# Aditya-Somasi/Vision-Inspection-System

Hardware: AMD Instinct MI355X
Metric: inspected images/sec (1024x1024, Qwen2-VL-7B) (higher is better)
Workload: dtype bf16; 1 GPU; configs[1]: Qwen2-VL-7B Inspector bf16, single 1024x1024 image per step per GPU, greedy decode 128 tok; batch=1, image_px=1024, weights=seeded random bf16 at exact 7B shapes, parallelism=dp1 (whole images)

## Files before the change

### vision-inspection-system_amd/csrc/decode.hip

```cpp
#include "decode_common.hip.h"
#include <stdlib.h>

template <int NB, bool AMAX, bool MASK>
__device__ __forceinline__ void gemv_bf16_body(GemvArgs p, const unsigned long long* __restrict__ allow) {
  extern __shared__ __attribute__((aligned(16))) char smem[];
  bf16_t* xs = (bf16_t*)smem;
  const int tid = threadIdx.x, lane = tid & 63, wave = tid >> 6;
  const int nch = p.K >> 3;

  const bool swiglu = (p.act == GV_ACT_SWIGLU);
  const int n_pairs = swiglu ? (p.N >> 1) : ((p.N + 1) >> 1);
  const int n_waves = gridDim.x * 4;
  const int wid = blockIdx.x * 4 + wave;
  const int p_begin = (int)((long long)n_pairs * wid / n_waves);
  const int p_end = (int)((long long)n_pairs * (wid + 1) / n_waves);
  const int nseg = ((nch + 63) / 64 + GV_SEG - 1) / GV_SEG;
  const int n_tasks = (p_end - p_begin) * nseg;

  GvBuf A, B;
  if (n_tasks > 0) gv_load(A, p, swiglu, p_begin, 0, lane, nch);

#pragma unroll
  for (int r = 0; r < NB; ++r) {
    if (r > 0) __syncthreads();
    gv_stage_row(p.x + (size_t)min(r, p.nb - 1) * p.ldx, p.norm_w, xs + (size_t)r * p.K, nch, p.K, p.eps, tid, lane, wave);
  }
  __syncthreads();

  float a0[NB], a1[NB];
#pragma unroll
  for (int r = 0; r < NB; ++r) { a0[r] = 0.f; a1[r] = 0.f; }
  float best = -INFINITY;
  int bi = 0x7fffffff;
  const unsigned am_step = AMAX ? (unsigned)*p.am_step : 0u;
  auto amax_rows = [&](int pr) {
    if (lane != 0) return;
    const int o = 2 * pr;
    float v0 = a0[0], v1 = a1[0];
    if (p.am_inv_temp > 0.f) {
      v0 = v0 * p.am_inv_temp + gumbel_noise(p.am_seed, am_step, (unsigned)o);
      v1 = v1 * p.am_inv_temp + gumbel_noise(p.am_seed, am_step, (unsigned)(o + 1));
    }
    bool ok0 = true, ok1 = true;
    if constexpr (MASK) {
      const unsigned long long m = allow[o >> 6];
      ok0 = (m >> (o & 63)) & 1ull;
      ok1 = (m >> ((o + 1) & 63)) & 1ull;
    }
    if (ok0 && (v0 > best || (v0 == best && o < bi))) { best = v0; bi = o; }
    if (ok1 && o + 1 < p.N && (v1 > best || (v1 == best && o + 1 < bi))) { best = v1; bi = o + 1; }
  };
  int pair = p_begin, seg = 0;
  for (int t = 0; t < n_tasks; t += 2) {
    int pair1 = pair, seg1 = seg + 1;
    if (seg1 == nseg) { seg1 = 0; ++pair1; }
    if (t + 1 < n_tasks) gv_load(B, p, swiglu, pair1, seg1, lane, nch);
    gv_consume<NB>(A, xs, p.K, seg, lane, nch, a0, a1);
    if (seg == nseg - 1) {
      gv_finish<NB>(p, swiglu, pair, lane, a0, a1);
      if constexpr (AMAX) amax_rows(pair);
#pragma unroll
      for (int r = 0; r < NB; ++r) { a0[r] = 0.f; a1[r] = 0.f; }
    }
    if (t + 1 >= n_tasks) break;
    int pair2 = pair1, seg2 = seg1 + 1;
    if (seg2 == nseg) { seg2 = 0; ++pair2; }
    if (t + 2 < n_tasks) gv_load(A, p, swiglu, pair2, seg2, lane, nch);
    gv_consume<NB>(B, xs, p.K, seg1, lane, nch, a0, a1);
    if (seg1 == nseg - 1) {
      gv_finish<NB>(p, swiglu, pair1, lane, a0, a1);
      if constexpr (AMAX) amax_rows(pair1);
#pragma unroll
      for (int r = 0; r < NB; ++r) { a0[r] = 0.f; a1[r] = 0.f; }
    }
    pair = pair2;
    seg = seg2;
  }
  if constexpr (AMAX) {
    __shared__ float am_v[4];
    __shared__ int am_i[4];
    if (lane == 0) { am_v[wave] = best; am_i[wave] = bi; }
    __syncthreads();
    if (tid == 0) {
      for (int w = 1; w < 4; ++w)
        if (am_v[w] > best || (am_v[w] == best && am_i[w] < bi)) { best = am_v[w]; bi = am_i[w]; }
      p.am_val[blockIdx.x] = best;
      p.am_idx[blockIdx.x] = bi;
    }
  }
}

template <int NB, bool AMAX = false>
__global__ __launch_bounds__(256) void gemv_bf16_kernel(GemvArgs p) { gemv_bf16_body<NB, AMAX, false>(p, nullptr); }

__global__ __launch_bounds__(256) void gemv_bf16_argmax_masked_kernel(GemvArgs p, const unsigned long long* allow) {
  gemv_bf16_body<1, true, true>(p, allow);
}

static int gemv_bf16_launch(GemvArgs p, hipStream_t stream) {
  const int n_pairs = (p.act == GV_ACT_SWIGLU) ? p.N / 2 : (p.N + 1) / 2;
  int blocks = (n_pairs + 3) / 4;
  if (blocks > 1024) blocks = 1024 + (blocks - 1024) / 8;
  if (blocks > 2048) blocks = 2048;
  vis_clear_error();
  if (p.nb == 1) {
    hipLaunchKernelGGL(gemv_bf16_kernel<1>, dim3(blocks), dim3(256), (size_t)p.K * 2, stream, p);
  } else {
    static const bool attr_ok = [] {
      return hipFuncSetAttribute((const void*)gemv_bf16_kernel<2>, hipFuncAttributeMaxDynamicSharedMemorySize, GV_ROWS_LDS_MAX) == hipSuccess &&
             hipFuncSetAttribute((const void*)gemv_bf16_kernel<4>, hipFuncAttributeMaxDynamicSharedMemorySize, GV_ROWS_LDS_MAX) == hipSuccess;
    }();
    if (!attr_ok) return VIS_ERR_LAUNCH;
    if (p.nb == 2) hipLaunchKernelGGL(gemv_bf16_kernel<2>, dim3(blocks), dim3(256), (size_t)p.K * 4, stream, p);
    else hipLaunchKernelGGL(gemv_bf16_kernel<4>, dim3(blocks), dim3(256), (size_t)p.K * 8, stream, p);
  }
  return vis_check_launch();
}

extern "C" int vis_gemv_bf16(const void* x, const void* W, const void* bias, const void* R, const void* norm_w,
                             void* y, int N, int K, int ldw, int act, int out_f32, float eps,
                             hipStream_t stream) {
  if (!x || !W || !y || N <= 0 || K <= 0) return VIS_ERR_ARG;
  if (K % 8 != 0 || ldw % 8 != 0 || K * 2 > 60 * 1024) return VIS_ERR_ARG;
  if (act != GV_ACT_NONE && act != GV_ACT_SWIGLU) return VIS_ERR_ARG;
  if (act == GV_ACT_SWIGLU && (N % 32 != 0 || bias || R || out_f32)) return VIS_ERR_ARG;
  if (((uintptr_t)x | (uintptr_t)W | (uintptr_t)norm_w) & 15) return VIS_ERR_ARG;
  GemvArgs p;
  p.x = (const bf16_t*)x; p.W = (const bf16_t*)W; p.bias = (const bf16_t*)bias; p.R = (const bf16_t*)R;
  p.norm_w = (const bf16_t*)norm_w; p.y = y;
  p.N = N; p.K = K; p.ldw = ldw; p.act = act; p.out_f32 = out_f32; p.eps = eps;
  p.outs_per_block = 0;
  p.nb = 1; p.ldx = 0; p.ldy = 0; p.ldr = 0;
  return gemv_bf16_launch(p, stream);
}

extern "C" int vis_gemv_bf16_rows(const void* x, const void* W, const void* bias, const void* R, const void* norm_w,
                                  void* y, int B, int N, int K, int ldw, int ldx, int ldy, int ldr, int act, int out_f32,
                                  float eps, hipStream_t stream) {
  if (!x || !W || !y || N <= 0 || K <= 0 || B < 1 || B > 4) return VIS_ERR_ARG;
  if (K % 8 != 0 || ldw % 8 != 0 || ldx % 8 != 0 || ldx < K) return VIS_ERR_ARG;
  const int nbk = (B == 1) ? 1 : (B == 2 ? 2 : 4);
  if ((size_t)K * 2 * nbk > (size_t)(nbk == 1 ? 60 * 1024 : GV_ROWS_LDS_MAX)) return VIS_ERR_ARG;
  if (act != GV_ACT_NONE && act != GV_ACT_SWIGLU) return VIS_ERR_ARG;
  if (act == GV_ACT_SWIGLU && (N % 32 != 0 || bias || R || out_f32)) return VIS_ERR_ARG;
  if (ldy < ((act == GV_ACT_SWIGLU) ? N / 2 : N) || (R && ldr < N)) return VIS_ERR_ARG;
  if (((uintptr_t)x | (uintptr_t)W | (uintptr_t)norm_w) & 15) return VIS_ERR_ARG;
  GemvArgs p;
  p.x = (const bf16_t*)x; p.W = (const bf16_t*)W; p.bias = (const bf16_t*)bias; p.R = (const bf16_t*)R;
  p.norm_w = (const bf16_t*)norm_w; p.y = y;
  p.N = N; p.K = K; p.ldw = ldw; p.act = act; p.out_f32 = out_f32; p.eps = eps;
  p.outs_per_block = 0;
  p.nb = B; p.ldx = ldx; p.ldy = ldy; p.ldr = ldr;
  return gemv_bf16_launch(p, stream);
}


struct GemvF8Args {
  const bf16_t* x;
  const uint8_t* W;
  const float* scale;
  const bf16_t* bias;
  const bf16_t* R;
  const bf16_t* norm_w;
  void* y;
  int N, K, ldw;
  int act, out_f32;
  float eps;
  int nb, ldx, ldy, ldr;
};

template <int ROWS, int SEG>
struct GfBuf {
  u32x4 w[ROWS][SEG];
};

template <int ROWS>
__device__ __forceinline__ void gf_rows(const GemvF8Args& p, bool swiglu, int quad, int* r) {
  if (swiglu) {
    const int o = (ROWS / 2) * quad;
    const int g0 = ((o >> 4) << 5) + (o & 15);
#pragma unroll
    for (int i = 0; i < ROWS / 2; ++i) { r[2 * i] = g0 + i; r[2 * i + 1] = g0 + 16 + i; }
  } else {
#pragma unroll
    for (int i = 0; i < ROWS; ++i) r[i] = min(ROWS * quad + i, p.N - 1);
  }
}

template <int ROWS, int SEG>
__device__ __forceinline__ void gf_load(GfBuf<ROWS, SEG>& b, const GemvF8Args& p, bool swiglu, int quad, int seg,
                                        int lane, int nch) {
  int r[ROWS];
  gf_rows<ROWS>(p, swiglu, quad, r);
#pragma unroll
  for (int i = 0; i < ROWS; ++i) {
    const uint8_t* w = p.W + (size_t)r[i] * p.ldw;
#pragma unroll
    for (int u = 0; u < SEG; ++u) {
      const int c = min(lane + 64 * (seg * SEG + u), nch - 1);
      b.w[i][u] = __builtin_nontemporal_load((const u32x4*)(w + c * 16));
    }
  }
}

struct Gf16 {
  bf16x2 v[8];
};
__device__ __forceinline__ Gf16 cvt16_f8(const u32x4& w) {
  Gf16 r;
#pragma unroll
  for (int i = 0; i < 4; ++i) {
    r.v[2 * i] = __builtin_amdgcn_cvt_scalef32_pk_bf16_fp8(w[i], 1.0f, false);
    r.v[2 * i + 1] = __builtin_amdgcn_cvt_scalef32_pk_bf16_fp8(w[i], 1.0f, true);
  }
  return r;
}
__device__ __forceinline__ float dot16_f8(const Gf16& w, const u32x4& xlo, const u32x4& xhi, float acc) {
  const bf16x8 xa = __builtin_bit_cast(bf16x8, xlo), xb = __builtin_bit_cast(bf16x8, xhi);
  acc = __builtin_amdgcn_fdot2_f32_bf16(w.v[0], __builtin_shufflevector(xa, xa, 0, 1), acc, false);
  acc = __builtin_amdgcn_fdot2_f32_bf16(w.v[1], __builtin_shufflevector(xa, xa, 2, 3), acc, false);
  acc = __builtin_amdgcn_fdot2_f32_bf16(w.v[2], __builtin_shufflevector(xa, xa, 4, 5), acc, false);
  acc = __builtin_amdgcn_fdot2_f32_bf16(w.v[3], __builtin_shufflevector(xa, xa, 6, 7), acc, false);
  acc = __builtin_amdgcn_fdot2_f32_bf16(w.v[4], __builtin_shufflevector(xb, xb, 0, 1), acc, false);
  acc = __builtin_amdgcn_fdot2_f32_bf16(w.v[5], __builtin_shufflevector(xb, xb, 2, 3), acc, false);
  acc = __builtin_amdgcn_fdot2_f32_bf16(w.v[6], __builtin_shufflevector(xb, xb, 4, 5), acc, false);
  acc = __builtin_amdgcn_fdot2_f32_bf16(w.v[7], __builtin_shufflevector(xb, xb, 6, 7), acc, false);
  return acc;
}

template <int ROWS, int SEG, int NB>
__device__ __forceinline__ void gf_consume(const GfBuf<ROWS, SEG>& b, const bf16_t* xs, int K, int seg, int lane, int nch,
                                           float (&a)[NB][ROWS]) {
#pragma unroll
  for (int u = 0; u < SEG; ++u) {
    const int c = lane + 64 * (seg * SEG + u);
    const int cc = min(c, nch - 1);
    u32x4 xlo[NB], xhi[NB];
#pragma unroll
    for (int r = 0; r < NB; ++r) {
      xlo[r] = *(const u32x4*)(xs + (size_t)r * K + cc * 16);
      xhi[r] = *(const u32x4*)(xs + (size_t)r * K + cc * 16 + 8);
      if (c >= nch) { xlo[r] = (u32x4){0u, 0u, 0u, 0u}; xhi[r] = xlo[r]; }
    }
#pragma unroll
    for (int i = 0; i < ROWS; ++i) {
      const Gf16 wv = cvt16_f8(b.w[i][u]);
#pragma unroll
      for (int r = 0; r < NB; ++r) a[r][i] = dot16_f8(wv, xlo[r], xhi[r], a[r][i]);
    }
  }
}

template <int ROWS, int NB>
__device__ __forceinline__ void gf_finish(const GemvF8Args& p, bool swiglu, int quad, int lane, float (&a)[NB][ROWS]) {
#pragma unroll
  for (int r = 0; r < NB; ++r)
#pragma unroll
    for (int i = 0; i < ROWS; ++i) a[r][i] = wave_sum(a[r][i]);
  if (lane != 0) return;
  int rw[ROWS];
  gf_rows<ROWS>(p, swiglu, quad, rw);
#pragma unroll
  for (int r = 0; r < NB; ++r) {
    if (r >= p.nb) break;
    if (swiglu) {
#pragma unroll
      for (int i = 0; i < ROWS / 2; ++i) {
        const float g = a[r][2 * i] * p.scale[rw[2 * i]], u = a[r][2 * i + 1] * p.scale[rw[2 * i + 1]];
        ((bf16_t*)p.y)[(size_t)r * p.ldy + (ROWS / 2) * quad + i] = f2bf(silu_fast(g) * u);
      }
      continue;
    }
#pragma unroll
    for (int i = 0; i < ROWS; ++i) {
      const int o = ROWS * quad + i;
      if (o >= p.N) break;
      float v = a[r][i] * p.scale[o];
      if (p.bias) v += bf2f(p.bias[o]);
      if (p.R) v += bf2f(p.R[(size_t)r * p.ldr + o]);
      if (p.out_f32) ((float*)p.y)[(size_t)r * p.ldy + o] = v;
      else ((bf16_t*)p.y)[(size_t)r * p.ldy + o] = f2bf(v);
    }
  }
}

template <int ROWS, int SEG, int NB>
__global__ __launch_bounds__(256) void gemv_fp8w_kernel(GemvF8Args p) {
  extern __shared__ __attribute__((aligned(16))) char smem[];
  bf16_t* xs = (bf16_t*)smem;
  const int tid = threadIdx.x, lane = tid & 63, wave = tid >> 6;
  const int nch8 = p.K >> 3;
  const int nch = p.K >> 4;
  const bool swiglu = (p.act == GV_ACT_SWIGLU);
  const int n_out = swiglu ? (p.N >> 1) : p.N;
  const int n_quads = swiglu ? (n_out / (ROWS / 2)) : ((n_out + ROWS - 1) / ROWS);
  const int n_waves = gridDim.x * 4;
  const int wid = blockIdx.x * 4 + wave;
  const int q_begin = (int)((long long)n_quads * wid / n_waves);
  const int q_end = (int)((long long)n_quads * (wid + 1) / n_waves);
  const int nseg = ((nch + 63) / 64 + SEG - 1) / SEG;
  const int n_tasks = (q_end - q_begin) * nseg;

  GfBuf<ROWS, SEG> A, B;
  if (n_tasks > 0) gf_load(A, p, swiglu, q_begin, 0, lane, nch);
// ... 550 lines not shown
}

__global__ __launch_bounds__(256) void argmax_stage1_kernel(const float* __restrict__ logits, int V,
                                                            float* __restrict__ bval, int* __restrict__ bidx,
                                                            float inv_temp, unsigned seed,
                                                            const int* __restrict__ step_ptr, int ld_logits) {
  argmax_stage1_body<false>(logits, V, bval, bidx, inv_temp, seed, step_ptr, ld_logits, nullptr, 0);
}

__global__ __launch_bounds__(256) void argmax_stage1_masked_kernel(const float* __restrict__ logits, int V,
                                                                   float* __restrict__ bval, int* __restrict__ bidx,
                                                                   float inv_temp, unsigned seed,
                                                                   const int* __restrict__ step_ptr, int ld_logits,
                                                                   const unsigned long long* __restrict__ allow,
                                                                   int ld_allow) {
  argmax_stage1_body<true>(logits, V, bval, bidx, inv_temp, seed, step_ptr, ld_logits, allow, ld_allow);
}

template <bool MASK>
__device__ __forceinline__ void argmax_stage2_body(const float* __restrict__ bval, const int* __restrict__ bidx, int nb,
                                                   int* __restrict__ tokens, int max_tokens, int* __restrict__ cur_token,
                                                   int* __restrict__ step_ptr) {
  const int lane = threadIdx.x, seq = blockIdx.x;
  bval += seq * 256;
  bidx += seq * 256;
  tokens += (size_t)seq * max_tokens;
  cur_token += seq;
  step_ptr += seq;
  float best = -INFINITY;
  int bi = 0x7fffffff;
  for (int i = lane; i < nb; i += 64) {
    const float v = bval[i];
    const int ix = bidx[i];
    if (v > best || (v == best && ix < bi)) { best = v; bi = ix; }
  }
#pragma unroll
  for (int o = 32; o > 0; o >>= 1) {
    const float ov = __shfl_xor(best, o, 64);
    const int oi = __shfl_xor(bi, o, 64);
    if (ov > best || (ov == best && oi < bi)) { best = ov; bi = oi; }
  }
  if (lane == 0) {
    if (MASK && bi == 0x7fffffff) bi = 0;
    const int st = *step_ptr;
    if (st < max_tokens) tokens[st] = bi;
    *cur_token = bi;
    *step_ptr = st + 1;
  }
}

__global__ __launch_bounds__(64) void argmax_stage2_kernel(const float* __restrict__ bval,
                                                           const int* __restrict__ bidx, int nb,
                                                           int* __restrict__ tokens, int max_tokens,
                                                           int* __restrict__ cur_token, int* __restrict__ step_ptr) {
  argmax_stage2_body<false>(bval, bidx, nb, tokens, max_tokens, cur_token, step_ptr);
}

__global__ __launch_bounds__(64) void argmax_stage2_masked_kernel(const float* __restrict__ bval,
                                                                  const int* __restrict__ bidx, int nb,
                                                                  int* __restrict__ tokens, int max_tokens,
                                                                  int* __restrict__ cur_token, int* __restrict__ step_ptr) {
  argmax_stage2_body<true>(bval, bidx, nb, tokens, max_tokens, cur_token, step_ptr);
}

extern "C" int vis_argmax_f32(const void* logits, int V, void* ws_val, void* ws_idx, void* tokens, int max_tokens,
                              void* cur_token, void* step_ptr, float inv_temp, unsigned seed, int batch,
                              int ld_logits, hipStream_t stream) {
  if (!logits || V <= 0 || !ws_val || !ws_idx || !tokens || !cur_token || !step_ptr) return VIS_ERR_ARG;
  if (!(inv_temp >= 0.f) || batch <= 0 || batch > 64 || (batch > 1 && ld_logits < V)) return VIS_ERR_ARG;
  const int nb = min(256, (V + 255) / 256);
  vis_clear_error();
  hipLaunchKernelGGL(argmax_stage1_kernel, dim3(nb, batch), dim3(256), 0, stream, (const float*)logits, V,
                     (float*)ws_val, (int*)ws_idx, inv_temp, seed, (const int*)step_ptr, ld_logits);
  hipLaunchKernelGGL(argmax_stage2_kernel, dim3(batch), dim3(64), 0, stream, (const float*)ws_val, (const int*)ws_idx,
                     nb, (int*)tokens, max_tokens, (int*)cur_token, (int*)step_ptr);
  return vis_check_launch();
}

extern "C" int vis_argmax_masked_f32(const void* logits, int V, void* ws_val, void* ws_idx, void* tokens, int max_tokens,
                                     void* cur_token, void* step_ptr, float inv_temp, unsigned seed, int batch,
                                     int ld_logits, const void* allow, int ld_allow, hipStream_t stream) {
  if (!logits || V <= 0 || !ws_val || !ws_idx || !tokens || !cur_token || !step_ptr || !allow) return VIS_ERR_ARG;
  if (!(inv_temp >= 0.f) || batch <= 0 || batch > 64 || (batch > 1 && ld_logits < V)) return VIS_ERR_ARG;
  if (ld_allow < (V + 63) / 64 || (((uintptr_t)allow) & 7)) return VIS_ERR_ARG;
  const int nb = min(256, (V + 255) / 256);
  vis_clear_error();
  hipLaunchKernelGGL(argmax_stage1_masked_kernel, dim3(nb, batch), dim3(256), 0, stream, (const float*)logits, V,
                     (float*)ws_val, (int*)ws_idx, inv_temp, seed, (const int*)step_ptr, ld_logits,
                     (const unsigned long long*)allow, ld_allow);
  hipLaunchKernelGGL(argmax_stage2_masked_kernel, dim3(batch), dim3(64), 0, stream, (const float*)ws_val,
                     (const int*)ws_idx, nb, (int*)tokens, max_tokens, (int*)cur_token, (int*)step_ptr);
  return vis_check_launch();
}

template <bool MASK>
__device__ __forceinline__ void argmax_merge_body(const float* __restrict__ bval, const int* __restrict__ bidx, int nb,
                                                  int* __restrict__ tokens, int max_tokens, int* __restrict__ cur_token,
                                                  int* __restrict__ step_ptr) {
  const int tid = threadIdx.x;
  float v[8];
  int ix[8];
#pragma unroll
  for (int k = 0; k < 8; ++k) {
    const int i = min(tid + 256 * k, nb - 1);
    v[k] = bval[i];
    ix[k] = bidx[i];
  }
  float best = -INFINITY;
  int bi = 0x7fffffff;
#pragma unroll
  for (int k = 0; k < 8; ++k)
    if (tid + 256 * k < nb && (v[k] > best || (v[k] == best && ix[k] < bi))) { best = v[k]; bi = ix[k]; }
#pragma unroll
  for (int o = 32; o > 0; o >>= 1) {
    const float ov = __shfl_xor(best, o, 64);
    const int oi = __shfl_xor(bi, o, 64);
    if (ov > best || (ov == best && oi < bi)) { best = ov; bi = oi; }
  }
  __shared__ float sv[4];
  __shared__ int si[4];
  if ((tid & 63) == 0) { sv[tid >> 6] = best; si[tid >> 6] = bi; }
  __syncthreads();
  if (tid == 0) {
    for (int w = 1; w < 4; ++w)
      if (sv[w] > best || (sv[w] == best && si[w] < bi)) { best = sv[w]; bi = si[w]; }
    if (MASK && bi == 0x7fffffff) bi = 0;
    const int st = *step_ptr;
    if (st < max_tokens) tokens[st] = bi;
    *cur_token = bi;
    *step_ptr = st + 1;
  }
}

__global__ __launch_bounds__(256) void argmax_merge_kernel(const float* __restrict__ bval, const int* __restrict__ bidx, int nb,
                                                           int* __restrict__ tokens, int max_tokens,
                                                           int* __restrict__ cur_token, int* __restrict__ step_ptr) {
  argmax_merge_body<false>(bval, bidx, nb, tokens, max_tokens, cur_token, step_ptr);
}

__global__ __launch_bounds__(256) void argmax_merge_masked_kernel(const float* __restrict__ bval, const int* __restrict__ bidx,
                                                                  int nb, int* __restrict__ tokens, int max_tokens,
                                                                  int* __restrict__ cur_token, int* __restrict__ step_ptr) {
  argmax_merge_body<true>(bval, bidx, nb, tokens, max_tokens, cur_token, step_ptr);
}

extern "C" int vis_gemv_bf16_argmax(const void* x, const void* W, const void* norm_w, void* logits, int N, int K, int ldw,
                                    float eps, void* ws_val, void* ws_idx, void* tokens, int max_tokens, void* cur_token,
                                    void* step_ptr, float inv_temp, unsigned seed, hipStream_t stream) {
  if (!x || !W || !logits || !ws_val || !ws_idx || !tokens || !cur_token || !step_ptr || N <= 0 || K <= 0) return VIS_ERR_ARG;
  if (K % 8 != 0 || ldw % 8 != 0 || K * 2 > 60 * 1024 || !(inv_temp >= 0.f)) return VIS_ERR_ARG;
  if (((uintptr_t)x | (uintptr_t)W | (uintptr_t)norm_w) & 15) return VIS_ERR_ARG;
  GemvArgs p;
  p.x = (const bf16_t*)x; p.W = (const bf16_t*)W; p.bias = nullptr; p.R = nullptr; p.norm_w = (const bf16_t*)norm_w;
  p.y = logits; p.N = N; p.K = K; p.ldw = ldw; p.act = GV_ACT_NONE; p.out_f32 = 1; p.eps = eps; p.outs_per_block = 0;
  p.nb = 1; p.ldx = 0; p.ldy = 0; p.ldr = 0;
  p.am_val = (float*)ws_val; p.am_idx = (int*)ws_idx; p.am_step = (const int*)step_ptr; p.am_inv_temp = inv_temp;
  p.am_seed = seed;
  const int n_pairs = (N + 1) / 2;
  int blocks = (n_pairs + 3) / 4;
  if (blocks > 1024) blocks = 1024 + (blocks - 1024) / 8;
  if (blocks > 2048) blocks = 2048;
  vis_clear_error();
  hipLaunchKernelGGL((gemv_bf16_kernel<1, true>), dim3(blocks), dim3(256), (size_t)K * 2, stream, p);
  hipLaunchKernelGGL(argmax_merge_kernel, dim3(1), dim3(256), 0, stream, (const float*)ws_val, (const int*)ws_idx, blocks,
                     (int*)tokens, max_tokens, (int*)cur_token, (int*)step_ptr);
  return vis_check_launch();
}

extern "C" int vis_gemv_bf16_argmax_masked(const void* x, const void* W, const void* norm_w, void* logits, int N, int K,
                                           int ldw, float eps, void* ws_val, void* ws_idx, void* tokens, int max_tokens,
                                           void* cur_token, void* step_ptr, float inv_temp, unsigned seed,
                                           const void* allow, hipStream_t stream) {
  if (!x || !W || !logits || !ws_val || !ws_idx || !tokens || !cur_token || !step_ptr || !allow || N <= 0 || K <= 0)
    return VIS_ERR_ARG;
  if (K % 8 != 0 || ldw % 8 != 0 || K * 2 > 60 * 1024 || !(inv_temp >= 0.f)) return VIS_ERR_ARG;
  if (((uintptr_t)x | (uintptr_t)W | (uintptr_t)norm_w) & 15 || (((uintptr_t)allow) & 7)) return VIS_ERR_ARG;
  GemvArgs p;
  p.x = (const bf16_t*)x; p.W = (const bf16_t*)W; p.bias = nullptr; p.R = nullptr; p.norm_w = (const bf16_t*)norm_w;
  p.y = logits; p.N = N; p.K = K; p.ldw = ldw; p.act = GV_ACT_NONE; p.out_f32 = 1; p.eps = eps; p.outs_per_block = 0;
  p.nb = 1; p.ldx = 0; p.ldy = 0; p.ldr = 0;
  p.am_val = (float*)ws_val; p.am_idx = (int*)ws_idx; p.am_step = (const int*)step_ptr; p.am_inv_temp = inv_temp;
  p.am_seed = seed;
  const int n_pairs = (N + 1) / 2;
  int blocks = (n_pairs + 3) / 4;
  if (blocks > 1024) blocks = 1024 + (blocks - 1024) / 8;
  if (blocks > 2048) blocks = 2048;
  vis_clear_error();
  hipLaunchKernelGGL(gemv_bf16_argmax_masked_kernel, dim3(blocks), dim3(256), (size_t)K * 2, stream, p,
                     (const unsigned long long*)allow);
  hipLaunchKernelGGL(argmax_merge_masked_kernel, dim3(1), dim3(256), 0, stream, (const float*)ws_val, (const int*)ws_idx,
                     blocks, (int*)tokens, max_tokens, (int*)cur_token, (int*)step_ptr);
  return vis_check_launch();
}
```

### vision-inspection-system_amd/csrc/decode_common.hip.h

```cpp
#pragma once
#include "common.hip.h"

typedef __bf16 bf16x2 __attribute__((ext_vector_type(2)));

enum { GV_ACT_NONE = 0, GV_ACT_SWIGLU = 3 };

struct GemvArgs {
  const bf16_t* x;
  const bf16_t* W;
  const bf16_t* bias;
  const bf16_t* R;
  const bf16_t* norm_w;
  void* y;
  int N, K, ldw;
  int act, out_f32;
  int outs_per_block;
  float eps;
  int nb, ldx, ldy, ldr;
  float* am_val;
  int* am_idx;
  const int* am_step;
  float am_inv_temp;
  unsigned am_seed;
};

__device__ __forceinline__ float gumbel_noise(unsigned seed, unsigned step, unsigned i) {
  unsigned long long z = ((unsigned long long)seed << 32) ^ ((unsigned long long)step * 0x9E3779B97F4A7C15ull) ^ i;
  z += 0x9E3779B97F4A7C15ull;
  z = (z ^ (z >> 30)) * 0xBF58476D1CE4E5B9ull;
  z = (z ^ (z >> 27)) * 0x94D049BB133111EBull;
  z ^= z >> 31;
  const float u = ((float)(z >> 41) + 0.5f) * (1.0f / 8388608.0f);
  return -__logf(-logf(u));
}



__device__ __forceinline__ float dot8(const u32x4& w, const u32x4& x, float acc) {
  const bf16x8 wv = __builtin_bit_cast(bf16x8, w), xv = __builtin_bit_cast(bf16x8, x);
  acc = __builtin_amdgcn_fdot2_f32_bf16(__builtin_shufflevector(wv, wv, 0, 1), __builtin_shufflevector(xv, xv, 0, 1), acc, false);
  acc = __builtin_amdgcn_fdot2_f32_bf16(__builtin_shufflevector(wv, wv, 2, 3), __builtin_shufflevector(xv, xv, 2, 3), acc, false);
  acc = __builtin_amdgcn_fdot2_f32_bf16(__builtin_shufflevector(wv, wv, 4, 5), __builtin_shufflevector(xv, xv, 4, 5), acc, false);
  acc = __builtin_amdgcn_fdot2_f32_bf16(__builtin_shufflevector(wv, wv, 6, 7), __builtin_shufflevector(xv, xv, 6, 7), acc, false);
  return acc;
}

#define GV_SEG 8

struct GvBuf {
  u32x4 w0[GV_SEG], w1[GV_SEG];
};

__device__ __forceinline__ void gv_rows(const GemvArgs& p, bool swiglu, int pair, int& r0, int& r1) {
  if (swiglu) {
    r0 = ((pair >> 4) << 5) + (pair & 15);
    r1 = r0 + 16;
  } else {
    r0 = 2 * pair;
    r1 = min(r0 + 1, p.N - 1);
  }
}

__device__ __forceinline__ void gv_load(GvBuf& b, const GemvArgs& p, bool swiglu, int pair, int seg, int lane,
                                        int nch) {
  int r0, r1;
  gv_rows(p, swiglu, pair, r0, r1);
  const bf16_t* w0 = p.W + (size_t)r0 * p.ldw;
  const bf16_t* w1 = p.W + (size_t)r1 * p.ldw;
#pragma unroll
  for (int u = 0; u < GV_SEG; ++u) {
    const int c = min(lane + 64 * (seg * GV_SEG + u), nch - 1);
    b.w0[u] = __builtin_nontemporal_load((const u32x4*)(w0 + c * 8));
    b.w1[u] = __builtin_nontemporal_load((const u32x4*)(w1 + c * 8));
  }
}

template <int NB>
__device__ __forceinline__ void gv_consume(const GvBuf& b, const bf16_t* xs, int K, int seg, int lane, int nch, float (&a0)[NB],
                                           float (&a1)[NB]) {
#pragma unroll
  for (int u = 0; u < GV_SEG; ++u) {
    const int c = lane + 64 * (seg * GV_SEG + u);
#pragma unroll
    for (int r = 0; r < NB; ++r) {
      u32x4 xv = *(const u32x4*)(xs + (size_t)r * K + min(c, nch - 1) * 8);
      if (c >= nch) xv = (u32x4){0u, 0u, 0u, 0u};
      a0[r] = dot8(b.w0[u], xv, a0[r]);
      a1[r] = dot8(b.w1[u], xv, a1[r]);
    }
  }
}

template <int NB>
__device__ __forceinline__ void gv_finish(const GemvArgs& p, bool swiglu, int pair, int lane, float (&a0)[NB], float (&a1)[NB]) {
#pragma unroll
  for (int r = 0; r < NB; ++r) {
    a0[r] = wave_sum(a0[r]);
    a1[r] = wave_sum(a1[r]);
  }
  if (lane != 0) return;
#pragma unroll
  for (int r = 0; r < NB; ++r) {
    if (r >= p.nb) break;
    if (swiglu) {
      ((bf16_t*)p.y)[(size_t)r * p.ldy + pair] = f2bf(silu_fast(a0[r]) * a1[r]);
      continue;
    }
    const int o = 2 * pair;
    const bool two = (o + 1 < p.N);
    float v0 = a0[r], v1 = a1[r];
    if (p.bias) { v0 += bf2f(p.bias[o]); if (two) v1 += bf2f(p.bias[o + 1]); }
    if (p.R) { v0 += bf2f(p.R[(size_t)r * p.ldr + o]); if (two) v1 += bf2f(p.R[(size_t)r * p.ldr + o + 1]); }
    if (p.out_f32) {
      ((float*)p.y)[(size_t)r * p.ldy + o] = v0;
      if (two) ((float*)p.y)[(size_t)r * p.ldy + o + 1] = v1;
    } else {
      ((bf16_t*)p.y)[(size_t)r * p.ldy + o] = f2bf(v0);
      if (two) ((bf16_t*)p.y)[(size_t)r * p.ldy + o + 1] = f2bf(v1);
    }
  }
}

template <bool SWZ>
__device__ __forceinline__ int gv_slot(int c) { return SWZ ? (c ^ ((c >> 4) & 3)) : c; }

#define GV_ROWS_LDS_MAX (152 * 1024)

template <bool SWZ = false>
__device__ __forceinline__ void gv_stage_x_rmsnorm(const bf16_t* __restrict__ x, const bf16_t* __restrict__ nw, bf16_t* xs,
                                                   int nch, int K, float eps, int tid, int lane, int wave) {
  __shared__ float red[4];
  if (nch <= 512) {
    const int c0 = tid, c1 = tid + 256;
    const u32x4 z = (u32x4){0u, 0u, 0u, 0u};
    const u32x4 r0 = (c0 < nch) ? *(const u32x4*)(x + c0 * 8) : z, r1 = (c1 < nch) ? *(const u32x4*)(x + c1 * 8) : z;
    const u32x4 g0 = (c0 < nch) ? *(const u32x4*)(nw + c0 * 8) : z, g1 = (c1 < nch) ? *(const u32x4*)(nw + c1 * 8) : z;
    float f0[8], f1[8], w0[8], w1[8], o[8];
    unpack8(r0, f0); unpack8(r1, f1);
    float ss = 0.f;
#pragma unroll
    for (int e = 0; e < 8; ++e) ss += f0[e] * f0[e] + f1[e] * f1[e];
    ss = wave_sum(ss);
    if (lane == 0) red[wave] = ss;
    __syncthreads();
    const float rstd = rsqrtf((red[0] + red[1] + red[2] + red[3]) / (float)K + eps);
    unpack8(g0, w0); unpack8(g1, w1);
    if (c0 < nch) {
#pragma unroll
      for (int e = 0; e < 8; ++e) o[e] = bf2f(f2bf(f0[e] * rstd)) * w0[e];
      *(u32x4*)(xs + gv_slot<SWZ>(c0) * 8) = pack8(o);
    }
    if (c1 < nch) {
#pragma unroll
      for (int e = 0; e < 8; ++e) o[e] = bf2f(f2bf(f1[e] * rstd)) * w1[e];
      *(u32x4*)(xs + gv_slot<SWZ>(c1) * 8) = pack8(o);
    }
    return;
  }
  float ss = 0.f;
  for (int c = tid; c < nch; c += 256) {
    float f[8];
    unpack8(*(const u32x4*)(x + c * 8), f);
#pragma unroll
    for (int e = 0; e < 8; ++e) ss += f[e] * f[e];
  }
  ss = wave_sum(ss);
  if (lane == 0) red[wave] = ss;
  __syncthreads();
  const float rstd = rsqrtf((red[0] + red[1] + red[2] + red[3]) / (float)K + eps);
// ... 371 lines not shown
```

Measured before the change: 2.647 images/s.

## Prefetch activation into registers and overlap with first weight loads in GEMV

Single-row GEMV kernels now load the activation vector into registers, issue the first two weight tile loads, and only then write the vector to LDS, fusing the RMSNorm for the argmax/LM-head path when K fits in two chunks per thread. Wide-K GEMVs without a norm (e.g. the MLP down projection, K=18944) get a 512-thread variant that stages more chunks per thread. This is meant to hide the activation staging latency behind weight prefetch in small-batch decode. In exchange it adds more template variants, more register pressure, and a wave count that is now passed in explicitly.

```diff
diff --git a/vision-inspection-system_amd/csrc/decode.hip b/vision-inspection-system_amd/csrc/decode.hip
--- a/vision-inspection-system_amd/csrc/decode.hip
+++ b/vision-inspection-system_amd/csrc/decode.hip
@@ -1,8 +1,11 @@
 #include "decode_common.hip.h"
 #include <stdlib.h>
 
-template <int NB, bool AMAX, bool MASK>
+template <int NB, bool AMAX, bool MASK, int NX, int NW>
 __device__ __forceinline__ void gemv_bf16_body(GemvArgs p, const unsigned long long* __restrict__ allow) {
+  static_assert(NB == 1 || NX == 0, "multi-row launches stage through gv_stage_row");
+  static_assert(NW == 4 || (NB == 1 && !AMAX && NX > 0), "the 512-thread form is the plain single-row kernel's");
+  constexpr int NT = 64 * NW;
   extern __shared__ __attribute__((aligned(16))) char smem[];
   bf16_t* xs = (bf16_t*)smem;
   const int tid = threadIdx.x, lane = tid & 63, wave = tid >> 6;
@@ -10,20 +13,77 @@
 
   const bool swiglu = (p.act == GV_ACT_SWIGLU);
   const int n_pairs = swiglu ? (p.N >> 1) : ((p.N + 1) >> 1);
-  const int n_waves = gridDim.x * 4;
-  const int wid = blockIdx.x * 4 + wave;
-  const int p_begin = (int)((long long)n_pairs * wid / n_waves);
-  const int p_end = (int)((long long)n_pairs * (wid + 1) / n_waves);
+  const int n_waves = p.n_waves;
+  const int wid = blockIdx.x * NW + wave;
+  const bool owns = NW == 4 || wid < n_waves;
+  const int p_begin = owns ? (int)((long long)n_pairs * wid / n_waves) : 0;
+  const int p_end = owns ? (int)((long long)n_pairs * (wid + 1) / n_waves) : 0;
   const int nseg = ((nch + 63) / 64 + GV_SEG - 1) / GV_SEG;
   const int n_tasks = (p_end - p_begin) * nseg;
 
   GvBuf A, B;
-  if (n_tasks > 0) gv_load(A, p, swiglu, p_begin, 0, lane, nch);
-
-#pragma unroll
-  for (int r = 0; r < NB; ++r) {
-    if (r > 0) __syncthreads();
-    gv_stage_row(p.x + (size_t)min(r, p.nb - 1) * p.ldx, p.norm_w, xs + (size_t)r * p.K, nch, p.K, p.eps, tid, lane, wave);
+  if constexpr (NB == 1 && NX > 0) {
+    const bool norm = NX == 2 && p.norm_w != nullptr;
+    u32x4 xv[NX], gw[2];
+    int xc[NX];
+#pragma unroll
+    for (int i = 0; i < NX; ++i) {
+      xc[i] = tid + i * NT;
+      xv[i] = *(const u32x4*)(p.x + (size_t)min(xc[i], nch - 1) * 8);
+    }
+    if constexpr (NX == 2) {
+      if (norm) {
+        gw[0] = *(const u32x4*)(p.norm_w + (size_t)min(xc[0], nch - 1) * 8);
+        gw[1] = *(const u32x4*)(p.norm_w + (size_t)min(xc[1], nch - 1) * 8);
+      }
+    }
+    const int pair0 = min(p_begin, n_pairs - 1);
+    const bool two = n_tasks > 1, nxt = nseg == 1;
+    gv_load(A, p, swiglu, pair0, 0, lane, nch);
+    gv_load(B, p, swiglu, (two && nxt) ? pair0 + 1 : pair0, (two && !nxt) ? 1 : 0, lane, nch);
+    bool plain = true;
+    if constexpr (NX == 2) {
+      if (norm) {
+        plain = false;
+        __shared__ float red[4];
+        const u32x4 z = (u32x4){0u, 0u, 0u, 0u};
+        u32x4 r0 = (xc[0] < nch) ? xv[0] : z, r1 = (xc[1] < nch) ? xv[1] : z;
+        float f0[8], f1[8], w0[8], w1[8], o[8];
+        unpack8(r0, f0); unpack8(r1, f1);
+        float ss = 0.f;
+#pragma unroll
+        for (int e = 0; e < 8; ++e) ss += f0[e] * f0[e] + f1[e] * f1[e];
+        ss = wave_sum(ss);
+        if (lane == 0) red[wave] = ss;
+        asm volatile("" : "+v"(r0), "+v"(r1));
+        __syncthreads();
+        const float rstd = rsqrtf((red[0] + red[1] + red[2] + red[3]) / (float)p.K + p.eps);
+        unpack8(r0, f0); unpack8(r1, f1);
+        unpack8(gw[0], w0); unpack8(gw[1], w1);
+        if (xc[0] < nch) {
+#pragma unroll
+          for (int e = 0; e < 8; ++e) o[e] = bf2f(f2bf(f0[e] * rstd)) * w0[e];
+          *(u32x4*)(xs + xc[0] * 8) = pack8(o);
+        }
+        if (xc[1] < nch) {
+#pragma unroll
+          for (int e = 0; e < 8; ++e) o[e] = bf2f(f2bf(f1[e] * rstd)) * w1[e];
+          *(u32x4*)(xs + xc[1] * 8) = pack8(o);
+        }
+      }
+    }
+    if (plain) {
+#pragma unroll
+      for (int i = 0; i < NX; ++i)
+        if (xc[i] < nch) *(u32x4*)(xs + xc[i] * 8) = xv[i];
+    }
+  } else {
+    if (n_tasks > 0) gv_load(A, p, swiglu, p_begin, 0, lane, nch);
+#pragma unroll
+    for (int r = 0; r < NB; ++r) {
+      if (r > 0) __syncthreads();
+      gv_stage_row(p.x + (size_t)min(r, p.nb - 1) * p.ldx, p.norm_w, xs + (size_t)r * p.K, nch, p.K, p.eps, tid, lane, wave);
+    }
   }
   __syncthreads();
 
@@ -54,7 +114,7 @@
   for (int t = 0; t < n_tasks; t += 2) {
     int pair1 = pair, seg1 = seg + 1;
     if (seg1 == nseg) { seg1 = 0; ++pair1; }
-    if (t + 1 < n_tasks) gv_load(B, p, swiglu, pair1, seg1, lane, nch);
+    if (t + 1 < n_tasks && (NX == 0 || t > 0)) gv_load(B, p, swiglu, pair1, seg1, lane, nch);
     gv_consume<NB>(A, xs, p.K, seg, lane, nch, a0, a1);
     if (seg == nseg - 1) {
       gv_finish<NB>(p, swiglu, pair, lane, a0, a1);
@@ -90,21 +150,38 @@
   }
 }
 
-template <int NB, bool AMAX = false>
-__global__ __launch_bounds__(256) void gemv_bf16_kernel(GemvArgs p) { gemv_bf16_body<NB, AMAX, false>(p, nullptr); }
-
+template <int NB, bool AMAX = false, int NX = 0, int NW = 4>
+__global__ __launch_bounds__(64 * NW) void gemv_bf16_kernel(GemvArgs p) { gemv_bf16_body<NB, AMAX, false, NX, NW>(p, nullptr); }
+
+template <int NX>
 __global__ __launch_bounds__(256) void gemv_bf16_argmax_masked_kernel(GemvArgs p, const unsigned long long* allow) {
-  gemv_bf16_body<1, true, true>(p, allow);
-}
-
-static int gemv_bf16_launch(GemvArgs p, hipStream_t stream) {
-  const int n_pairs = (p.act == GV_ACT_SWIGLU) ? p.N / 2 : (p.N + 1) / 2;
+  gemv_bf16_body<1, true, true, NX, 4>(p, allow);
+}
+
+static int gemv_bf16_blocks(int n_pairs) {
   int blocks = (n_pairs + 3) / 4;
   if (blocks > 1024) blocks = 1024 + (blocks - 1024) / 8;
   if (blocks > 2048) blocks = 2048;
+  return blocks;
+}
+
+static int gemv_bf16_nx(int K, int threads, bool norm) {
+  const int need = ((K >> 3) + threads - 1) / threads;
+  if (norm && need > 2) return 0;
+  return need <= 2 ? 2 : need <= 5 ? 5 : 10;
+}
+
+static int gemv_bf16_launch(GemvArgs p, hipStream_t stream) {
+  const int n_pairs = (p.act == GV_ACT_SWIGLU) ? p.N / 2 : (p.N + 1) / 2;
+  const int blocks = gemv_bf16_blocks(n_pairs);
+  p.n_waves = blocks * 4;
   vis_clear_error();
   if (p.nb == 1) {
-    hipLaunchKernelGGL(gemv_bf16_kernel<1>, dim3(blocks), dim3(256), (size_t)p.K * 2, stream, p);
+    const size_t lds = (size_t)p.K * 2;
+    const bool wide = p.K > 8192 && !p.norm_w;
+    if (!wide) hipLaunchKernelGGL((gemv_bf16_kernel<1, false, 0, 4>), dim3(blocks), dim3(256), lds, stream, p);
+    else if (gemv_bf16_nx(p.K, 512, false) == 5) hipLaunchKernelGGL((gemv_bf16_kernel<1, false, 5, 8>), dim3((blocks + 1) / 2), dim3(512), lds, stream, p);
+    else hipLaunchKernelGGL((gemv_bf16_kernel<1, false, 10, 8>), dim3((blocks + 1) / 2), dim3(512), lds, stream, p);
   } else {
     static const bool attr_ok = [] {
       return hipFuncSetAttribute((const void*)gemv_bf16_kernel<2>, hipFuncAttributeMaxDynamicSharedMemorySize, GV_ROWS_LDS_MAX) == hipSuccess &&
@@ -129,7 +206,7 @@
   p.x = (const bf16_t*)x; p.W = (const bf16_t*)W; p.bias = (const bf16_t*)bias; p.R = (const bf16_t*)R;
   p.norm_w = (const bf16_t*)norm_w; p.y = y;
   p.N = N; p.K = K; p.ldw = ldw; p.act = act; p.out_f32 = out_f32; p.eps = eps;
-  p.outs_per_block = 0;
+  p.n_waves = 0;
   p.nb = 1; p.ldx = 0; p.ldy = 0; p.ldr = 0;
   return gemv_bf16_launch(p, stream);
 }
@@ -149,7 +226,7 @@
   p.x = (const bf16_t*)x; p.W = (const bf16_t*)W; p.bias = (const bf16_t*)bias; p.R = (const bf16_t*)R;
   p.norm_w = (const bf16_t*)norm_w; p.y = y;
   p.N = N; p.K = K; p.ldw = ldw; p.act = act; p.out_f32 = out_f32; p.eps = eps;
-  p.outs_per_block = 0;
+  p.n_waves = 0;
   p.nb = B; p.ldx = ldx; p.ldy = ldy; p.ldr = ldr;
   return gemv_bf16_launch(p, stream);
 }
@@ -1006,16 +1083,15 @@
   if (((uintptr_t)x | (uintptr_t)W | (uintptr_t)norm_w) & 15) return VIS_ERR_ARG;
   GemvArgs p;
   p.x = (const bf16_t*)x; p.W = (const bf16_t*)W; p.bias = nullptr; p.R = nullptr; p.norm_w = (const bf16_t*)norm_w;
-  p.y = logits; p.N = N; p.K = K; p.ldw = ldw; p.act = GV_ACT_NONE; p.out_f32 = 1; p.eps = eps; p.outs_per_block = 0;
+  p.y = logits; p.N = N; p.K = K; p.ldw = ldw; p.act = GV_ACT_NONE; p.out_f32 = 1; p.eps = eps; p.n_waves = 0;
   p.nb = 1; p.ldx = 0; p.ldy = 0; p.ldr = 0;
   p.am_val = (float*)ws_val; p.am_idx = (int*)ws_idx; p.am_step = (const int*)step_ptr; p.am_inv_temp = inv_temp;
   p.am_seed = seed;
-  const int n_pairs = (N + 1) / 2;
-  int blocks = (n_pairs + 3) / 4;
-  if (blocks > 1024) blocks = 1024 + (blocks - 1024) / 8;
-  if (blocks > 2048) blocks = 2048;
+  const int blocks = gemv_bf16_blocks((N + 1) / 2);
+  p.n_waves = blocks * 4;
   vis_clear_error();
-  hipLaunchKernelGGL((gemv_bf16_kernel<1, true>), dim3(blocks), dim3(256), (size_t)K * 2, stream, p);
+  if (gemv_bf16_nx(K, 256, true) == 2) hipLaunchKernelGGL((gemv_bf16_kernel<1, true, 2, 4>), dim3(blocks), dim3(256), (size_t)K * 2, stream, p);
+  else hipLaunchKernelGGL((gemv_bf16_kernel<1, true, 0, 4>), dim3(blocks), dim3(256), (size_t)K * 2, stream, p);
   hipLaunchKernelGGL(argmax_merge_kernel, dim3(1), dim3(256), 0, stream, (const float*)ws_val, (const int*)ws_idx, blocks,
                      (int*)tokens, max_tokens, (int*)cur_token, (int*)step_ptr);
   return vis_check_launch();
@@ -1031,17 +1107,17 @@
   if (((uintptr_t)x | (uintptr_t)W | (uintptr_t)norm_w) & 15 || (((uintptr_t)allow) & 7)) return VIS_ERR_ARG;
   GemvArgs p;
   p.x = (const bf16_t*)x; p.W = (const bf16_t*)W; p.bias = nullptr; p.R = nullptr; p.norm_w = (const bf16_t*)norm_w;
-  p.y = logits; p.N = N; p.K = K; p.ldw = ldw; p.act = GV_ACT_NONE; p.out_f32 = 1; p.eps = eps; p.outs_per_block = 0;
+  p.y = logits; p.N = N; p.K = K; p.ldw = ldw; p.act = GV_ACT_NONE; p.out_f32 = 1; p.eps = eps; p.n_waves = 0;
   p.nb = 1; p.ldx = 0; p.ldy = 0; p.ldr = 0;
   p.am_val = (float*)ws_val; p.am_idx = (int*)ws_idx; p.am_step = (const int*)step_ptr; p.am_inv_temp = inv_temp;
   p.am_seed = seed;
-  const int n_pairs = (N + 1) / 2;
-  int blocks = (n_pairs + 3) / 4;
-  if (blocks > 1024) blocks = 1024 + (blocks - 1024) / 8;
-  if (blocks > 2048) blocks = 2048;
+  const int blocks = gemv_bf16_blocks((N + 1) / 2);
+  p.n_waves = blocks * 4;
   vis_clear_error();
-  hipLaunchKernelGGL(gemv_bf16_argmax_masked_kernel, dim3(blocks), dim3(256), (size_t)K * 2, stream, p,
-                     (const unsigned long long*)allow);
+  if (gemv_bf16_nx(K, 256, true) == 2)
+    hipLaunchKernelGGL(gemv_bf16_argmax_masked_kernel<2>, dim3(blocks), dim3(256), (size_t)K * 2, stream, p, (const unsigned long long*)allow);
+  else
+    hipLaunchKernelGGL(gemv_bf16_argmax_masked_kernel<0>, dim3(blocks), dim3(256), (size_t)K * 2, stream, p, (const unsigned long long*)allow);
   hipLaunchKernelGGL(argmax_merge_masked_kernel, dim3(1), dim3(256), 0, stream, (const float*)ws_val, (const int*)ws_idx,
                      blocks, (int*)tokens, max_tokens, (int*)cur_token, (int*)step_ptr);
   return vis_check_launch();
diff --git a/vision-inspection-system_amd/csrc/decode_common.hip.h b/vision-inspection-system_amd/csrc/decode_common.hip.h
--- a/vision-inspection-system_amd/csrc/decode_common.hip.h
+++ b/vision-inspection-system_amd/csrc/decode_common.hip.h
@@ -14,7 +14,7 @@
   void* y;
   int N, K, ldw;
   int act, out_f32;
-  int outs_per_block;
+  int n_waves;
   float eps;
   int nb, ldx, ldy, ldr;
   float* am_val;
```

After: 2.672 images/s, median of 6. Within noise of the previous version (+0.9%).
